# tristanGIANDO/python_ray_tracer

Measured on AMD Instinct MI355X. Metric: Mpixels/sec @1920x1080, 3 reflection bounces, higher is better.
Workload: dtype f64; 1 GPU; C2: README scene (BASELINE configs[1]) 1920x1080, 3 bounces; width=1920, height=1080, max_bounces=3, spheres=3, output=f32, mode=frames, parallelism=framesx1

## Files before the change

python_ray_tracer_amd/csrc/rtx_device.h:

```cpp
#pragma once

#include <hip/hip_ext.h>
#include <hip/hip_runtime.h>

#include <cstdint>
#include <cstdio>
#include <cstdlib>
#include <cstring>

#include "../../include/rtx_hip.h"
#include "rtx_internal.h"

#define FARAWAY 1.0e39
#define RTX_PI 3.141592653589793

namespace {

constexpr int kBlock = 256;
constexpr int kWaveW = 8;
constexpr int kWaveWSmall = 16;
constexpr int kFastWaves = 4;
constexpr int kFastWavesSmall = 1;
constexpr int kPersistMinSpheres = 32;
constexpr int kMaxFetch = 32;
constexpr int kDeferredWorkers = 4096;
constexpr int kDeepWorkers = 16384;
constexpr int kDeepWaves = 4;
constexpr int kDeepWavesTile = 5;
constexpr int kFwdWavesPersist = 4;
constexpr int kFwdWaves = 5;
constexpr int kFwdWavesLarge = 6;
constexpr int64_t kWavesLargeMinPixels = int64_t(4) << 20;
constexpr int kFwdWavesSmall = 5;
constexpr int kDeepLevels = 5;
constexpr int kCappedMax = RTX_FAST_MAX_BOUNCES;
constexpr int kShadeMath = 3;
constexpr int kWaveH = 64 / kWaveW;
static_assert(kFastWaves == 1 || kFastWaves == 2 || kFastWaves == 4, "kFastWaves");
static_assert(kFastWavesSmall == 1 || kFastWavesSmall == 2 || kFastWavesSmall == 4, "kFastWavesSmall");
static_assert((kMaxFetch & (kMaxFetch - 1)) == 0, "kMaxFetch must be a power of two");
constexpr int kFastBlock = 64 * kFastWaves;
constexpr int kWavesX = kFastWavesSmall == 1 ? 1 : 2;
constexpr int kWavesXTree = kFastWaves;
static_assert(kWaveWSmall > 0 && kWaveWSmall <= 64 && 64 % kWaveWSmall == 0, "kWaveWSmall");
template <bool TREE>
__host__ __device__ constexpr int wave_w() { return TREE ? kWaveW : kWaveWSmall; }
template <bool TREE>
__host__ __device__ constexpr int waves_x() { return TREE ? kWavesXTree : kWavesX; }
template <bool TREE>
__host__ __device__ constexpr int fast_waves() { return TREE ? kFastWaves : kFastWavesSmall; }
template <bool TREE>
// ... 40 lines not shown
  int64_t n_workers;
  int stack_levels;
  unsigned long long* stats;
  int n_tiles_x, n_tiles_y;
  uint32_t* fetch;
  int n_fetch;
  int64_t scene_stride;
  int n_frames;
  int frame;
  uint32_t* deferred_out;
  int no_general;
  int images;
  const uint32_t* tile_order;
  uint32_t* tile_cost;
  int reserve;
};

constexpr int kFrameShift = 34;
constexpr int kRaysShift = 50;
constexpr int kHitsShift = 57;
constexpr int kLevelMask = 0x7F;
constexpr int kRecWords = 10;
constexpr int kFirstPassLevels = 30;
constexpr int kDeepLevel3 = 60;
static_assert(kFirstPassLevels >= kDeepLevels && kFirstPassLevels < kDeepLevel3, "first-pass record level");
static_assert(kDeepLevel3 + 2 < kLevelMask, "deferred-entry level fields hold 7 bits");
constexpr int64_t records_cap(int64_t n, bool cont) {
  const int64_t lo = int64_t(1) << (cont ? 14 : 18);
  const int64_t by_n = n / (cont ? 2048 : 32);
  const int64_t want = by_n > lo ? by_n : lo;
// ... 19 lines not shown
}

__device__ __forceinline__ Params frame_view(const Params& p, int f) {
  Params q = p;
  q.scene = p.scene + (int64_t)f * p.scene_stride;
  q.out = (uint8_t*)p.out + (int64_t)f * p.n * out_bytes_per_pixel(p.out_kind);
  q.frame = f;
  return q;
}


__device__ __forceinline__ double dot3(double ax, double ay, double az, double bx, double by, double bz) {
  return ((ax * bx) + (ay * by)) + (az * bz);
}

__device__ __forceinline__ double sqrt_core(double x) {
  const double y = __builtin_amdgcn_rsq(x);
  double g = x * y;
  double h = y * 0.5;
  const double r = __builtin_fma(-h, g, 0.5);
  g = __builtin_fma(g, r, g);
  h = __builtin_fma(h, r, h);
  double d = __builtin_fma(-g, g, x);
  g = __builtin_fma(d, h, g);
  d = __builtin_fma(-g, g, x);
  return __builtin_fma(d, h, g);
}
__device__ __forceinline__ double sqrt_cr(double x) {
  if (__ballot(!(x >= 0x1.0p-767 && x <= 0x1.fffffffffffffp+1023)) == 0) return sqrt_core(x);
  return __builtin_sqrt(x);
// ... 6 lines not shown
  r = __builtin_fma(r, e, r);
  const double q = a * r;
  const double rem = __builtin_fma(-b, q, a);
  return __builtin_fma(rem, r, q);
}
__device__ __forceinline__ bool div_range(double x) {
  const double ax = fabs(x);
  return ax >= 0x1.0p-300 && ax <= 0x1.0p+300;
}
__device__ __forceinline__ double div_cr(double a, double b) {
  if (__ballot(!(div_range(b) && (a == 0.0 || div_range(a)))) == 0)
    return a == 0.0 ? a * __builtin_copysign(1.0, b) : div_core(a, b);
  return a / b;
}

__device__ __forceinline__ double inv_mag(double d) {
  if (__ballot(!(d >= 0x1.0p-600 && d <= 0x1.0p+600)) == 0) return div_core(1.0, sqrt_core(d));
  const double mag = sqrt_cr(d);
  return div_cr(1.0, mag == 0.0 ? 1.0 : mag);
}

__device__ __forceinline__ void norm3(double& x, double& y, double& z) {
  const double r = inv_mag(dot3(x, y, z, x, y, z));
  x = x * r;
  y = y * r;
  z = z * r;
}

__device__ __forceinline__ double inv_mag_near1(double d) {
  return __builtin_fma(-__builtin_floor((d - 1.0) * 0x1.0p51), 0x1.0p-52, 1.0);
}
__device__ __forceinline__ double inv_mag_unit(double d) {
  if (__ballot(!(fabs(d - 1.0) <= 0x1.0p-30)) == 0) return inv_mag_near1(d);
  return inv_mag(d);
}
__device__ __forceinline__ void norm3_unit(double& x, double& y, double& z) {
  const double r = inv_mag_unit(dot3(x, y, z, x, y, z));
  x = x * r;
  y = y * r;
  z = z * r;
}

__device__ __forceinline__ double clip01(double x) { return __builtin_fmin(__builtin_fmax(x, 0.0), 1.0); }

__device__ __forceinline__ double max0(double x) { return __builtin_fmax(x, 0.0); }

__device__ __forceinline__ int trunc_parity(double x) {
  const double k = trunc(x);
  const double h = k * 0.5;
  return (x == x) && (h != trunc(h));
}

// ... 12 lines not shown
  if (disc > 0.0 && !behind(b, c)) {
    const double sq = sqrt_cr(disc);
    const double s0 = (-b - sq) * 0.5;
    const double s1 = (-b + sq) * 0.5;
    const double sol = s0 > 0.0 ? s0 : s1;
    if (sol > 0.0) t = sol;
  }
  return t;
}

struct SphTest {
  double h, d;
  bool skip;
  int half;
};
__device__ __forceinline__ SphTest sph_test(double h, double c, double tame) {
  SphTest t;
  t.half = __ballot(!(fabs(h) >= tame)) == 0 ? 1 : 0;
  t.h = h;
  if (t.half) {
    t.d = (h * h) - c;
    t.skip = !(t.d > 0.0) || (h > 0.0 && c >= 0.0);
  } else {
    const double b = 2.0 * h;
    t.d = (b * b) - (4.0 * c);
    t.skip = !(t.d > 0.0) || behind(b, c);
  }
  return t;
}
template <typename P>
__device__ __forceinline__ SphTest isect_disc(const P* g, double ox, double oy, double oz, double oo, double dx,
                                              double dy, double dz, double tame) {
  const double cx = g[RTX_G_CX], cy = g[RTX_G_CY], cz = g[RTX_G_CZ];
  const double h = dot3(dx, dy, dz, ox - cx, oy - cy, oz - cz);
  const double c = ((g[RTX_G_CC] + oo) - 2.0 * dot3(cx, cy, cz, ox, oy, oz)) - g[RTX_G_RR];
  return sph_test(h, c, tame);
}
template <typename P>
__device__ __forceinline__ SphTest isect_disc_cam(const P* g, double ox, double oy, double oz, double dx, double dy,
                                                  double dz, double tame) {
  const double h = dot3(dx, dy, dz, ox - g[RTX_G_CX], oy - g[RTX_G_CY], oz - g[RTX_G_CZ]);
  return sph_test(h, g[RTX_G_C0], tame);
}
__device__ __forceinline__ double isect_sol(const SphTest& t, bool& valid) {
  if (t.half) {
    const double sq = sqrt_core(fabs(t.d));
    valid = !t.skip && sq > t.h;
    const uint32_t hi = __double2hiint(sq), lo = __double2loint(sq);
    const uint32_t shi = (-t.h > sq) ? (hi ^ 0x80000000u) : hi;
    return -t.h + __hiloint2double(shi, lo);
  }
  const double b = 2.0 * t.h;
  const double sq = sqrt_cr(fabs(t.d));
  const double s0 = (-b - sq) * 0.5;
  const double s1 = (-b + sq) * 0.5;
// ... 5 lines not shown
  if (!a.skip) {
    bool v;
    const double t = isect_sol(a, v);
    f(t, v);
  }
}
template <typename F>
__device__ __forceinline__ void isect_pair(const SphTest& a, const SphTest& b, F&& f) {
  if (!a.skip || !b.skip) {
    bool v0, v1;
    const double t0 = isect_sol(a, v0);
    const double t1 = isect_sol(b, v1);
    f(t0, v0, t1, v1);
  }
}
template <typename P>
__device__ __forceinline__ double isect_t(const P* g, double ox, double oy, double oz, double oo, double dx, double dy,
                                          double dz, double tame) {
  double r = FARAWAY;
  isect_one(isect_disc(g, ox, oy, oz, oo, dx, dy, dz, tame), [&](double t, bool v) {
    if (v) r = t;
  });
  return r;
}

__device__ __forceinline__ void nearest_update(bool valid, double t, int s, double& tmin, int& hit, bool& tie) {
  if (valid && t < tmin) {
    tmin = t;
    hit = s;
    tie = false;
  } else if (valid && t == tmin) {
    tie = true;
  }
// ... 193 lines not shown
          const cdouble* g0 = cg + __builtin_amdgcn_readfirstlane(k) * RTX_GEOM_WORDS;
          isect_one(isect_disc(g0, qx, qy, qz, qq, lx, ly, lz, tame), [&](double t0, bool v0) {
            if (v0 && t0 < tself) lit = false;
          });
        }
      }
      if (__ballot(lit) == 0) break;
      ++i;
    } else {
      i = (int)nd[RTX_N_SKIP];
    }
  }
  return lit;
}

template <bool CAM, typename P, typename Wk>
__device__ __forceinline__ void nearest_hit(const P* geo, int nsph, double ox, double oy, double oz, double dx,
                                            double dy, double dz, double& tmin, int& hit, bool& tie, double tame,
                                            Wk& wk) {
  wk.test(nsph);
  tmin = FARAWAY;
  hit = -1;
  tie = false;
  const double oo = CAM ? 0.0 : dot3(ox, oy, oz, ox, oy, oz);
  scan_range(
      geo, 0, nsph,
      [&](const P* g) {
        return CAM ? isect_disc_cam(g, ox, oy, oz, dx, dy, dz, tame) : isect_disc(g, ox, oy, oz, oo, dx, dy, dz, tame);
      },
      [](const P*, int s) { return s; }, [&](int s, double t, bool v) { nearest_update(v, t, s, tmin, hit, tie); });
}

__device__ __forceinline__ double sin_reduced(double x) {
// ... 3 lines not shown
  r = __builtin_fma(-n, -0x1.f1976b7ed8fbcp-109, r);
  const double z = r * r;
  double q = 0x1.71b8ef6dcf572p-66;
  q = __builtin_fma(z, q, -0x1.2f49b46814157p-57);
  q = __builtin_fma(z, q, 0x1.952c77030ad4ap-49);
  q = __builtin_fma(z, q, -0x1.ae7f3e733b81fp-41);
  q = __builtin_fma(z, q, 0x1.6124613a86d09p-33);
  q = __builtin_fma(z, q, -0x1.ae64567f544e4p-26);
  q = __builtin_fma(z, q, 0x1.71de3a556c734p-19);
  q = __builtin_fma(z, q, -0x1.a01a01a01a01ap-13);
  q = __builtin_fma(z, q, 0x1.1111111111111p-7);
  q = __builtin_fma(z, q, -0x1.5555555555555p-3);
  const double s = __builtin_fma(r * z, q, r);
  return ((int)n & 1) ? -s : s;
}
__device__ __forceinline__ double sin_ref(const cdouble* sc, double x) {
  if (sc[RTX_H_SINRED] != 0.0 || __ballot(!(fabs(x) <= 0x1.0p20)) == 0) return sin_reduced(x);
  return sin(x);
}

__device__ __forceinline__ double div_shade(double a, double b) {
  if constexpr (kShadeMath == 0) return div_cr(a, b);
  if constexpr (kShadeMath == 1) return div_core(a, b);
  double r = __builtin_amdgcn_rcp(b);
  r = __builtin_fma(r, __builtin_fma(-b, r, 1.0), r);
  r = __builtin_fma(r, __builtin_fma(-b, r, 1.0), r);
  return a * r;
}
__device__ __forceinline__ double sqrt_shade(double x) {
  if constexpr (kShadeMath == 0) return sqrt_cr(x);
  if constexpr (kShadeMath == 1) return x == 0.0 ? 0.0 : sqrt_core(x);
// ... 48 lines not shown
}

struct Hit {
  double dli;
  double di;
  double spec;
  double va;
  double g;
  int h;
  int tk;
  bool lit;
  double qx, qy, qz;
  double nx, ny, nz;
};

template <typename M>
__device__ __forceinline__ double specular(const M* mh, double g, double nx, double ny, double nz, double lx,
                                           double ly, double lz, double vx, double vy, double vz) {
  double Lx = lx, Ly = ly, Lz = lz;
  norm3_unit(Lx, Ly, Lz);
  double Vx = vx, Vy = vy, Vz = vz;
  norm3_unit(Vx, Vy, Vz);
  double Hx = Lx + Vx, Hy = Ly + Vy, Hz = Lz + Vz;
  {
    const double dh = dot3(Hx, Hy, Hz, Hx, Hy, Hz);
    const double rh = kShadeMath == 4 ? inv_mag_shade(dh) : inv_mag_shade_v(dh);
    Hx = Hx * rh;
    Hy = Hy * rh;
    Hz = Hz * rh;
  }
  const double NdotV = clip01(dot3(nx, ny, nz, Vx, Vy, Vz));
  if (!(NdotV > 0.0)) return 0.0;
  const double NdotH = clip01(dot3(nx, ny, nz, Hx, Hy, Hz));
  const double VdotH = clip01(dot3(Vx, Vy, Vz, Hx, Hy, Hz));
  const double NdotL = clip01(dot3(nx, ny, nz, Lx, Ly, Lz));
  const double F = __builtin_fma(mh[RTX_M_1MF0], pow5(1.0 - VdotH), mh[RTX_M_F0]);
  const double a2 = mh[RTX_M_A2];
  const double denom = (NdotH * NdotH) * mh[RTX_M_A2M1] + 1.0;
  const double Dd = RTX_PI * __builtin_fma(denom, denom, 1e-8);
  const double oma2 = mh[RTX_M_1MA2];
  const double dL = (NdotL + sqrt_shade(__builtin_fma(oma2, NdotL * NdotL, a2))) + 1e-8;
  const double dV = (NdotV + sqrt_shade(__builtin_fma(oma2, NdotV * NdotV, a2))) + 1e-8;
  const double spec_base = ((F * a2) * ((2.0 * NdotL) * (2.0 * NdotV))) *
                           div_shade(1.0, (dL * dV) * (Dd * __builtin_fma(4.0, NdotV, 1e-8)));
  const double glint = pow25(1.0 - NdotV) * NdotL;
  const double sf = __builtin_fma(g, glint, spec_base);
  return (NdotV <= 0.0) ? 0.0 : sf;
}

template <bool IMG = false, typename M>
__device__ __forceinline__ void hit_color(const M* mh, const cdouble* sc, double dli, double di, int tk, bool lit,
                                          bool weighted, double spec, double va, double Rr, double Rg, double Rb,
                                          double& cr, double& cg, double& cb) {
  const double litf = lit ? 1.0 : 0.0;
  double tr, tg, tb;
  const double tex = mh[RTX_M_TEX];
  if (tex == RTX_TEX_CHECKER) {
    tr = tg = tb = tk ? 1.0 : 0.0;
  } else if (IMG && tex == RTX_TEX_IMAGE) {
    const cdouble* t = sc + ((int64_t)mh[RTX_M_TR] + 3 * (int64_t)tk);
    tr = t[0];
    tg = t[1];
    tb = t[2];
  } else {
    tr = mh[RTX_M_TR];
    tg = mh[RTX_M_TG];
    tb = mh[RTX_M_TB];
  }
  const double dg = mh[RTX_M_DG];
  const double ar = __builtin_fma(sc[RTX_H_DOMEC + 0], di, __builtin_fma((tr * dli) * litf, dg, 0.004));
  const double ag = __builtin_fma(sc[RTX_H_DOMEC + 1], di, __builtin_fma((tg * dli) * litf, dg, 0.004));
  const double ab = __builtin_fma(sc[RTX_H_DOMEC + 2], di, __builtin_fma((tb * dli) * litf, dg, 0.004));
  const double g = mh[RTX_M_G];
  const double xr = weighted ? (spec + Rr * 0.5) * g : 0.0;
  const double xg = weighted ? (spec + Rg * 0.5) * g : 0.0;
  const double xb = weighted ? (spec + Rb * 0.5) * g : 0.0;
  double ir = 0.0, ig = 0.0, ib = 0.0;
  const double igain = mh[RTX_M_IG];
  if (igain != 0.0) {
    const double af = fabs(va - 0.5) * 2.0;
    const double phase = ((af * RTX_PI) * mh[RTX_M_TFT]) * 10.0;
    const double ip = sin_ref(sc, phase);
    const double hs = mh[RTX_M_HS], omhs = mh[RTX_M_1MHS];
    const double r = __builtin_fma(ip, hs, omhs * (1.0 - ip));
    const double gg = __builtin_fma(ip, omhs, hs * (1.0 - ip));
    const double b = __builtin_fma(0.5, ip, 0.5);
    const double w = mh[RTX_M_TFW];
    ir = (r * w) * igain;
    ig = (gg * w) * igain;
    ib = (b * w) * igain;
  }
  cr = (ar + xr) + ir;
  cg = (ag + xg) + ig;
  cb = (ab + xb) + ib;
}

constexpr int kGridWaterfall = 16;
// ... 53 lines not shown
                   [&](double t0, bool v0, double t1, bool v1) {
                     if (v0) tsh = __builtin_fmin(tsh, t0);
                     if (v1) tsh = __builtin_fmin(tsh, t1);
                     anyv = anyv || v0 || v1;
                   });
      } else {
        isect_one(a0, [&](double t0, bool v0) {
          if (v0) tsh = __builtin_fmin(tsh, t0);
          anyv = anyv || v0;
        });
      }
    }
  }
}

template <bool IMG = false, bool TREE = true, typename T, typename G, typename Wk>
__device__ __forceinline__ void shade(const cdouble* sc, const G* geo, const T* tab, int nsph, int h, double ox,
                                      double oy, double oz, double dx, double dy, double dz, double t, Hit& s,
                                      double tame, Wk& wk, const T* mat = nullptr) {
  const T* gh = tab + h * RTX_GEOM_WORDS;
  const T* mh = mat ? mat : tab + nsph * RTX_GEOM_WORDS + h * RTX_MAT_WORDS;
  const double px = ox + dx * t, py = oy + dy * t, pz = oz + dz * t;
  const double inv_r = gh[RTX_G_INVR];
  const double nx = (px - gh[RTX_G_CX]) * inv_r;
  const double ny = (py - gh[RTX_G_CY]) * inv_r;
  const double nz = (pz - gh[RTX_G_CZ]) * inv_r;
  double lx = sc[RTX_H_LIGHT + 0] - px, ly = sc[RTX_H_LIGHT + 1] - py, lz = sc[RTX_H_LIGHT + 2] - pz;
  norm3(lx, ly, lz);
  const double qx = px + nx * 0.0001, qy = py + ny * 0.0001, qz = pz + nz * 0.0001;

  const double qq = dot3(qx, qy, qz, qx, qy, qz);
  const int h0 = __builtin_amdgcn_readfirstlane(h);
  const int hs = __ballot(h != h0) == 0 ? h0 : nsph;
  bool lit = true;
  uint64_t m0, m1;
  if (TREE && sc[RTX_H_SHGRID] != 0.0 && sc[RTX_H_TAME] != 0.0 &&
      grid_mask(sc, qx, qy, qz, qq, lx, ly, lz, dot3(nx, ny, nz, nx, ny, nz), hs, m0, m1)) {
    wk.node();
    if ((m0 | m1) != 0) {
      double tsh;
      bool anyv;
      min_masked(geo, m0, m1, qx, qy, qz, qq, lx, ly, lz, tame, tsh, anyv, wk);
      if (__ballot(anyv) != 0) {
        const double tself = isect_t(gh, qx, qy, qz, qq, lx, ly, lz, tame);
        wk.test(1);
        lit = !(anyv && tsh < tself);
      }
    }
  } else if (!TREE && sc[RTX_H_TAME] != 0.0) {
    const int nshadow = nsph - (hs < nsph);
    double tsh = FARAWAY;
    bool anyv = false;
    int j = 0;
    for (; j + 1 < nshadow; j += 2) {
      const G* g0 = geo + __builtin_amdgcn_readfirstlane(j + (j >= hs)) * RTX_GEOM_WORDS;
      const G* g1 = geo + __builtin_amdgcn_readfirstlane(j + 1 + (j + 1 >= hs)) * RTX_GEOM_WORDS;
      wk.test(2);
      isect_pair(isect_disc(g0, qx, qy, qz, qq, lx, ly, lz, tame), isect_disc(g1, qx, qy, qz, qq, lx, ly, lz, tame),
                 [&](double t0, bool v0, double t1, bool v1) {
                   if (v0) tsh = __builtin_fmin(tsh, t0);
                   if (v1) tsh = __builtin_fmin(tsh, t1);
                   anyv = anyv || v0 || v1;
                 });
    }
// ... 50 lines not shown
  double di = 0.0;
  for (int j = 0; j < ndome; ++j) di = di + sc[RTX_H_DOMEI + j] * max0(up);

  const double g = mh[RTX_M_G];
  const bool weighted = lit && g != 0.0;
  const bool need_irid = mh[RTX_M_IG] != 0.0;
  double spec = 0.0, va = 0.0;
  if (weighted || need_irid) {
    double vx = sc[RTX_H_CAM + 0] - px, vy = sc[RTX_H_CAM + 1] - py, vz = sc[RTX_H_CAM + 2] - pz;
    {
      const double rv = inv_mag_shade_v(dot3(vx, vy, vz, vx, vy, vz));
      vx = vx * rv;
      vy = vy * rv;
      vz = vz * rv;
    }
    if (weighted) spec = specular(mh, g, nx, ny, nz, lx, ly, lz, vx, vy, vz);
    if (need_irid) va = clip01(dot3(nx, ny, nz, vx, vy, vz));
  }
  s.dli = dli;
  s.di = di;
  s.spec = spec;
  s.va = va;
  s.g = g;
  s.h = h;
  const double tex = mh[RTX_M_TEX];
  s.tk = tex == RTX_TEX_CHECKER ? (trunc_parity(px * 2.0) == trunc_parity(pz * 2.0))
         : tex != RTX_TEX_IMAGE ? 0
         : IMG ? image_texel(mh, gh, px, py, pz) : -1;
  s.lit = lit;
  s.qx = qx; s.qy = qy; s.qz = qz;
  s.nx = nx; s.ny = ny; s.nz = nz;
}

__device__ __forceinline__ void reflect_dir(double& dx, double& dy, double& dz, double nx, double ny, double nz) {
  const double dn = dot3(dx, dy, dz, nx, ny, nz);
  double rx = dx - (nx * 2.0) * dn, ry = dy - (ny * 2.0) * dn, rz = dz - (nz * 2.0) * dn;
  norm3_unit(rx, ry, rz);
  dx = rx;
  dy = ry;
  dz = rz;
}


__device__ __forceinline__ int global_row(const Params& p, int lr) {
  if (p.n_parts == 1) return lr;
  const int own = p.row_block * p.part_run;
  return (lr / own) * (p.n_parts * p.row_block) + p.part * p.row_block + (lr % own);
}

__device__ __forceinline__ void camera_dir(const cdouble* sc, int col, int r, int W, int H, double& dx, double& dy,
                                           double& dz) {
  const double x = (sc[RTX_H_XFIX] != 0.0 && col == W - 1) ? sc[RTX_H_XSTOP]
                                                            : (double)col * sc[RTX_H_XSTEP] + sc[RTX_H_XSTART];
  const double y = (sc[RTX_H_YFIX] != 0.0 && r == H - 1) ? sc[RTX_H_YSTOP]
                                                          : (double)r * sc[RTX_H_YSTEP] + sc[RTX_H_YSTART];
  const double vx = x - sc[RTX_H_CAM + 0];
  const double vy = y - sc[RTX_H_CAM + 1];
  const double vz = sc[RTX_H_VZ];
  const double rr = inv_mag(((vx * vx) + (vy * vy)) + sc[RTX_H_VZ2]);
  dx = vx * rr;
  dy = vy * rr;
  dz = vz * rr;
}

__device__ __forceinline__ void camera_ray(const Params& p, int col, int lr, double& ox, double& oy, double& oz,
                                           double& dx, double& dy, double& dz) {
  const cdouble* sc = (const cdouble*)p.scene;
  camera_dir(sc, col, global_row(p, lr), p.width, p.height, dx, dy, dz);
  ox = sc[RTX_H_CAM + 0];
  oy = sc[RTX_H_CAM + 1];
  oz = sc[RTX_H_CAM + 2];
}

__device__ __forceinline__ int huge_tail(const cdouble* sc, int nsph) {
  const int nb = (int)sc[RTX_H_NBEAM];
  return nb > 0 && nb < nsph ? nb : nsph;
}

__device__ __forceinline__ bool wave_frustum(const Params& p, int c0, int lr0, uint64_t& m0, uint64_t& m1) {
  const cdouble* sc = (const cdouble*)p.scene;
  const int W = p.width;
  if (c0 >= W || lr0 >= p.n_rows) return false;
  const int c1 = c0 + kWaveW - 1 < W - 1 ? c0 + kWaveW - 1 : W - 1;
// ... 244 lines not shown
    o[1] = quant_u8(g);
    o[2] = quant_u8(b);
  }
}

__device__ __forceinline__ void stat_add(unsigned long long* st, int word, unsigned long long v) {
  atomicAdd(st + word, v);
}

__device__ __forceinline__ void stat_wave(unsigned long long* st, int word) {
  const unsigned long long m = __ballot(1);
  if ((int)__lane_id() == __ffsll((long long)m) - 1) atomicAdd(st + word, 1ull);
}


template <int B, bool LDS, int DEEP, bool STATS, bool TREE, bool BEAM, bool IMG = false, int NSPH = 0>
__device__ __forceinline__ void fast_tile(const Params& p, int bx, int by, bool first, const double* lds_tab,
                                          bool wave_tile = false) {
  constexpr int FB = fast_block<TREE>();
  const cdouble* sc = (const cdouble*)p.scene;
  const cdouble* geo = sc + RTX_HDR_WORDS;
  const int nsph = NSPH > 0 ? NSPH : p.nsph;
  const int nb = TREE ? huge_tail(sc, nsph) : nsph;
  const double tame = p.mode != 1 && p.mode != 3 && sc[RTX_H_TAME] != 0.0 ? 0x1.0p-350 : __builtin_nan("");

  int64_t i = 0;
  bool active;
  int kb = 0;
  const double* rin = nullptr;
  int col = 0, lr = 0;
  constexpr int WW = wave_w<TREE>(), WH = 64 / WW, WX = waves_x<TREE>(), WY = fast_waves<TREE>() / WX;
  const int wv = __builtin_amdgcn_readfirstlane((int)(threadIdx.x >> 6));
  auto pixel_index = [&](int lane) -> int64_t {
    if (p.mode == 0) {
      const int c = wave_tile ? bx * WW + (lane % WW) : bx * (WX * WW) + (wv % WX) * WW + (lane % WW);
      const int r = wave_tile ? by * WH + (lane / WW) : by * (WY * WH) + (wv / WX) * WH + (lane / WW);
      return (int64_t)r * p.width + c;
    }
    return (int64_t)bx * FB + wv * 64 + lane;
// ... 33 lines not shown
  uint64_t fm0 = 0, fm1 = 0;
  bool fr = false;
  if constexpr (TREE) {
    if (cam0 && nsph <= 128 && sc[RTX_H_NNODES] != 0.0 && sc[RTX_H_SBOX] != 0.0 && sc[RTX_H_TAME] != 0.0 &&
        sc[RTX_H_VZ] != 0.0) {
      const int lane = threadIdx.x & 63;
      fr = wave_frustum(p, __builtin_amdgcn_readfirstlane(col - lane % kWaveW),
                        __builtin_amdgcn_readfirstlane(lr - lane / kWaveW), fm0, fm1);
    }
  }
  if (active) {
    if (rin) {
      ox = rin[0]; oy = rin[1]; oz = rin[2];
      dx = rin[3]; dy = rin[4]; dz = rin[5];
    } else if (cam0) {
      camera_ray(p, col, lr, ox, oy, oz, dx, dy, dz);
    } else {
      load_ray(p, i, ox, oy, oz, dx, dy, dz);
    }
    if (st) {
      if (!rin) stat_add(st, RTX_S_PIXELS, 1);
      if (kb < RTX_S_LEVELS) {
        stat_add(st, RTX_S_RAYS + kb, 1);
        stat_wave(st, RTX_S_WTRACE + kb);
      }
    }
    if (p.mode == 3) {
      tmin = p.hit_t[i];
      hit = p.hit_shape;
      tie = sc[RTX_H_MAT0] != 0.0;
    } else if (TREE && sc[RTX_H_NNODES] != 0.0) {
      if (fr) {
        nearest_masked<true>(geo, fm0, fm1, ox, oy, oz, dx, dy, dz, tmin, hit, tie, tame, wk);
      } else if (cam0) {
        nearest_bvh<true>(sc, ox, oy, oz, dx, dy, dz, tmin, hit, tie, tame, wk);
      } else {
        nearest_bvh<false>(sc, ox, oy, oz, dx, dy, dz, tmin, hit, tie, tame, wk);
      }
    } else if (cam0) {
      nearest_hit<true>(geo, nsph, ox, oy, oz, dx, dy, dz, tmin, hit, tie, tame, wk);
    } else {
      nearest_hit<false>(geo, nsph, ox, oy, oz, dx, dy, dz, tmin, hit, tie, tame, wk);
    }
  }
  if constexpr (LDS) {
    if (first) __syncthreads();
  }
  if (!active) return;
  constexpr bool CL = !DEEP && LDS && TREE && !BEAM;
  static_assert(!CL || 3 * sizeof(double) * FB == kColourLdsBytes, "colour LDS");
  double* const cl = CL ? const_cast<double*>(lds_tab) + nsph * kSphWords + threadIdx.x : nullptr;
  if constexpr (CL) {
    cl[0] = 0.0;
    cl[FB] = 0.0;
    cl[2 * FB] = 0.0;
  }

  double cr = 0.0, cg = 0.0, cb = 0.0;
  double thr = 1.0;
  if constexpr (DEEP == 2) {
    if (rin) {
      cr = rin[6];
      cg = rin[7];
// ... 23 lines not shown
      deferred = true;
      rays_through = kb + k;
      hits_through = kb + k - 1;
      break;
    }
    if (st && kb + k < RTX_S_LEVELS) {
      stat_add(st, RTX_S_HITS + kb + k, 1);
      stat_wave(st, RTX_S_WSHADE + kb + k);
    }
    const bool weighted = s.lit && s.g != 0.0;
    const bool at_cap = DEEP && p.max_bounces >= 0 && kb + k >= p.max_bounces;
    {
      const double* tab = LDS ? (const double*)lds_tab : p.scene + RTX_HDR_WORDS;
      double lr_, lg_, lb_;
      hit_color<IMG>(tab + nsph * RTX_GEOM_WORDS + hit * RTX_MAT_WORDS, sc, s.dli, s.di, s.tk, s.lit, weighted, s.spec,
                     s.va, 0.0, 0.0, 0.0, lr_, lg_, lb_);
      if constexpr (CL) {
        cl[0] = __builtin_fma(thr, lr_, cl[0]);
        cl[FB] = __builtin_fma(thr, lg_, cl[FB]);
        cl[2 * FB] = __builtin_fma(thr, lb_, cl[2 * FB]);
      } else {
        cr = __builtin_fma(thr, lr_, cr);
        cg = __builtin_fma(thr, lg_, cg);
        cb = __builtin_fma(thr, lb_, cb);
      }
      const int kmax = DEEP ? p.drec_level - kb : B;
      if (DEEP && weighted && k >= kmax && !at_cap) {
        deferred = true;
        appended = true;
        rays_through = hits_through = kb + kmax;
        const int64_t slot = append_deferred(p, deferred_entry(DEEP == 2 || !TREE ? i : pixel_index(lane_id_fresh()),
                                                               p.frame, kb + kmax, kb + kmax));
        if (p.drec && slot >= 0 && slot < p.rec_cap) {
          double* rec = p.drec + slot * kRecWords;
          double rx = dx, ry = dy, rz = dz;
          reflect_dir(rx, ry, rz, s.nx, s.ny, s.nz);
          rec[0] = s.qx; rec[1] = s.qy; rec[2] = s.qz;
          rec[3] = rx; rec[4] = ry; rec[5] = rz;
          rec[6] = cr; rec[7] = cg; rec[8] = cb;
          rec[9] = (thr * 0.5) * s.g;
        }
        break;
      }
      if (!weighted || k >= kmax || at_cap) break;
      thr = (thr * 0.5) * s.g;
    }
    reflect_dir(dx, dy, dz, s.nx, s.ny, s.nz);
    ox = s.qx;
    oy = s.qy;
    oz = s.qz;
    if (st && kb + k + 1 < RTX_S_LEVELS) {
      stat_add(st, RTX_S_RAYS + kb + k + 1, 1);
      stat_wave(st, RTX_S_WTRACE + kb + k + 1);
    }
    [[maybe_unused]] uint32_t tests0 = 0, nodes0 = 0;
    if constexpr (STATS) {
      tests0 = wk.tests;
      nodes0 = wk.nodes;
    }
    if (TREE && sc[RTX_H_NNODES] != 0.0) {
      Beam bm;
      const double* btab = LDS ? (const double*)lds_tab : p.scene + RTX_HDR_WORDS;
// ... 11 lines not shown
      wk.tests1 += wk.tests - tests0;
      wk.nodes1 += wk.nodes - nodes0;
    }
  }

  if constexpr (STATS) {
    if (st) {
      stat_add(st, RTX_S_TESTS, wk.tests);
      stat_add(st, RTX_S_NODES, wk.nodes);
      stat_add(st, RTX_S_TESTS1, wk.tests1);
      stat_add(st, RTX_S_NODES1, wk.nodes1);
      stat_add(st, RTX_S_BOXES, wk.boxes);
      stat_add(st, RTX_S_BEAMT, wk.beamt);
    }
  }
  const int64_t io = DEEP == 2 || !TREE ? i : pixel_index(lane_id_fresh());
  if constexpr (CL) {
    cr = cl[0];
    cg = cl[FB];
    cb = cl[2 * FB];
  }
  if (deferred) {
    if (!appended) append_deferred(p, deferred_entry(io, p.frame, rays_through, hits_through));
    if (st && !rin) stat_add(st, RTX_S_DEFERRED, 1);
    return;
  }
  write_out(p, io, cr, cg, cb);
}

template <int B, bool LDS, int DEEP, bool STATS, int TP, bool IMG, int NSPH>
__device__ __forceinline__ void k_render_fast_tiles(const Params& p, const double* lds_tab);

template <int B, bool LDS, int DEEP, bool STATS = false, int TP = 2, bool IMG = false, int NSPH = 0, int WAVES = 0>
__global__ __launch_bounds__(fast_block<(TP >= 1)>(),
                             WAVES > 0 ? WAVES
                             : DEEP    ? (TP >= 2 || DEEP == 2 ? kDeepWaves : kDeepWavesTile)
                                       : (TP >= 2 ? kFwdWavesPersist : TP ? kFwdWaves : kFwdWavesSmall)) void
k_render_fast(Params p0) {
  constexpr bool TREE = TP >= 1;
  constexpr bool BEAM = TP >= 2;
  extern __shared__ double lds_tab[];
  const Params p = frame_view(p0, blockIdx.z);
  {
    const cdouble* sc = (const cdouble*)p.scene;
    if (sc[RTX_H_MAGIC] != RTX_MAGIC || sc[RTX_H_NSPH] != (double)p.nsph || (NSPH > 0 && p.nsph != NSPH)) {
      if (threadIdx.x == 0) atomicOr((uint32_t*)p.ws + RTX_WS_STATUS, (uint32_t)RTX_ST_BAD_SCENE);
      return;
    }
  }
  if constexpr (LDS) {
    const double* src = p.scene + RTX_HDR_WORDS;
    for (int k = threadIdx.x; k < p.nsph * kSphWords; k += fast_block<TREE>()) {
      const bool bw = BEAM && kBeamStaged && k < p.nsph * RTX_GEOM_WORDS && (k & (RTX_GEOM_WORDS - 1)) == RTX_G_IDX;
      lds_tab[k] = bw ? beam_word(src[k - RTX_G_IDX + RTX_G_CC], src[k - RTX_G_IDX + RTX_G_RR]) : src[k];
    }
  }
  if constexpr (DEEP == 2) {
// ... 47 lines not shown
    return;
  }
  const uint64_t t_entry = STATS && p.tile_cost ? __builtin_amdgcn_s_memrealtime() : 0;
  int bx = blockIdx.x, by = gridDim.y - 1 - blockIdx.y, tb = blockIdx.y * gridDim.x + blockIdx.x;
  if (p.tile_order) {
    tb = (int)((const uint32_t __attribute__((address_space(4)))*)p.tile_order)[tb];
    if ((unsigned)tb >= gridDim.x * gridDim.y) return;
    bx = tb % gridDim.x;
    by = gridDim.y - 1 - tb / gridDim.x;
  }
  fast_tile<B, LDS, DEEP, STATS, TREE, BEAM, IMG, NSPH>(p, bx, by, true, lds_tab);
  if (STATS && p.tile_cost && (threadIdx.x & 63) == 0)
    atomicMax(p.tile_cost + tb, (uint32_t)(__builtin_amdgcn_s_memrealtime() - t_entry));
}

}
```

python_ray_tracer_amd/csrc/rtx_small.hip:

```cpp
#include "rtx_device.h"
#include "rtx_internal.h"

namespace {

template <int B, int DEEP, bool STATS, bool IMG = false, int NSPH = 0>
hipError_t go(const void* params, dim3 grid, uint32_t lds, hipStream_t s, hipEvent_t e0, hipEvent_t e1) {
  const Params& p = *static_cast<const Params*>(params);
  rtx_note_launch(B, true, DEEP, STATS, 0, IMG, NSPH, 0, grid, p.n_fetch, p.tile_order != nullptr, lds);
  hipExtLaunchKernelGGL((k_render_fast<B, true, DEEP, STATS, 0, IMG, NSPH>), grid, dim3(fast_block<false>()), lds, s,
                        e0, e1, 0u, p);
  return hipSuccess;
}

template <int B, int DEEP>
hipError_t go_ns(const void* params, dim3 grid, uint32_t lds, hipStream_t s, hipEvent_t e0, hipEvent_t e1) {
  static_assert(kTreeMinSpheres == 8, "one instantiation per sphere count 1..7");
  switch (static_cast<const Params*>(params)->nsph) {
    case 1: return go<B, DEEP, false, false, 1>(params, grid, lds, s, e0, e1);
    case 2: return go<B, DEEP, false, false, 2>(params, grid, lds, s, e0, e1);
    case 3: return go<B, DEEP, false, false, 3>(params, grid, lds, s, e0, e1);
    case 4: return go<B, DEEP, false, false, 4>(params, grid, lds, s, e0, e1);
    case 5: return go<B, DEEP, false, false, 5>(params, grid, lds, s, e0, e1);
    case 6: return go<B, DEEP, false, false, 6>(params, grid, lds, s, e0, e1);
    case 7: return go<B, DEEP, false, false, 7>(params, grid, lds, s, e0, e1);
// ... 35 lines not shown
```

Before: 42320 Mpixels/s.

## Add optimistic small-scene wave path with sticky range guards and deferred LDS staging

Adds a dedicated small_wave path for single-wave small-scene kernels. It runs an optimistic tile body in which the per-call wave ballots for range checks (sqrt/div/normalise, sphere test, sine reduction) become a sticky per-lane flag; if any lane trips it, the whole tile is recomputed with the exact path. Scene table words are preloaded into registers and written to LDS only when some lane actually hits a sphere, and tile_order decoding uses a precomputed reciprocal instead of division. This trades fewer ballots and branches for higher register pressure, more code, and a possible full redo on rare inputs.

```diff
diff --git a/python_ray_tracer_amd/csrc/rtx_device.h b/python_ray_tracer_amd/csrc/rtx_device.h
--- a/python_ray_tracer_amd/csrc/rtx_device.h
+++ b/python_ray_tracer_amd/csrc/rtx_device.h
@@ -7,6 +7,7 @@
 #include <cstdio>
 #include <cstdlib>
 #include <cstring>
+#include <type_traits>
 
 #include "../../include/rtx_hip.h"
 #include "rtx_internal.h"
@@ -35,6 +36,8 @@
 constexpr int kDeepLevels = 5;
 constexpr int kCappedMax = RTX_FAST_MAX_BOUNCES;
 constexpr int kShadeMath = 3;
+constexpr bool kSmallOptimistic = true;
+constexpr bool kSmallLateStage = true;
 constexpr int kWaveH = 64 / kWaveW;
 static_assert(kFastWaves == 1 || kFastWaves == 2 || kFastWaves == 4, "kFastWaves");
 static_assert(kFastWavesSmall == 1 || kFastWavesSmall == 2 || kFastWavesSmall == 4, "kFastWavesSmall");
@@ -105,6 +108,7 @@
   const uint32_t* tile_order;
   uint32_t* tile_cost;
   int reserve;
+  uint32_t tile_div;
 };
 
 constexpr int kFrameShift = 34;
@@ -154,6 +158,14 @@
   return ((ax * bx) + (ay * by)) + (az * bz);
 }
 
+struct Sticky {
+  bool& bad;
+  __device__ __forceinline__ operator double() const { return 0x1.0p-350; }
+  __device__ __forceinline__ void trip(bool failed) const { bad = bad || failed; }
+};
+template <typename Tm>
+constexpr bool kSticky = std::is_same<Tm, Sticky>::value;
+
 __device__ __forceinline__ double sqrt_core(double x) {
   const double y = __builtin_amdgcn_rsq(x);
   double g = x * y;
@@ -190,14 +202,20 @@
   return a / b;
 }
 
-__device__ __forceinline__ double inv_mag(double d) {
+template <typename Tm = double>
+__device__ __forceinline__ double inv_mag(double d, Tm tame = Tm()) {
+  if constexpr (kSticky<Tm>) {
+    tame.trip(!(d >= 0x1.0p-600 && d <= 0x1.0p+600));
+    return div_core(1.0, sqrt_core(d));
+  }
   if (__ballot(!(d >= 0x1.0p-600 && d <= 0x1.0p+600)) == 0) return div_core(1.0, sqrt_core(d));
   const double mag = sqrt_cr(d);
   return div_cr(1.0, mag == 0.0 ? 1.0 : mag);
 }
 
-__device__ __forceinline__ void norm3(double& x, double& y, double& z) {
-  const double r = inv_mag(dot3(x, y, z, x, y, z));
+template <typename Tm = double>
+__device__ __forceinline__ void norm3(double& x, double& y, double& z, Tm tame = Tm()) {
+  const double r = inv_mag(dot3(x, y, z, x, y, z), tame);
   x = x * r;
   y = y * r;
   z = z * r;
@@ -206,12 +224,18 @@
 __device__ __forceinline__ double inv_mag_near1(double d) {
   return __builtin_fma(-__builtin_floor((d - 1.0) * 0x1.0p51), 0x1.0p-52, 1.0);
 }
-__device__ __forceinline__ double inv_mag_unit(double d) {
+template <typename Tm = double>
+__device__ __forceinline__ double inv_mag_unit(double d, Tm tame = Tm()) {
+  if constexpr (kSticky<Tm>) {
+    tame.trip(!(fabs(d - 1.0) <= 0x1.0p-30));
+    return inv_mag_near1(d);
+  }
   if (__ballot(!(fabs(d - 1.0) <= 0x1.0p-30)) == 0) return inv_mag_near1(d);
   return inv_mag(d);
 }
-__device__ __forceinline__ void norm3_unit(double& x, double& y, double& z) {
-  const double r = inv_mag_unit(dot3(x, y, z, x, y, z));
+template <typename Tm = double>
+__device__ __forceinline__ void norm3_unit(double& x, double& y, double& z, Tm tame = Tm()) {
+  const double r = inv_mag_unit(dot3(x, y, z, x, y, z), tame);
   x = x * r;
   y = y * r;
   z = z * r;
@@ -254,9 +278,15 @@
   bool skip;
   int half;
 };
-__device__ __forceinline__ SphTest sph_test(double h, double c, double tame) {
+template <typename Tm>
+__device__ __forceinline__ SphTest sph_test(double h, double c, Tm tame) {
   SphTest t;
-  t.half = __ballot(!(fabs(h) >= tame)) == 0 ? 1 : 0;
+  if constexpr (kSticky<Tm>) {
+    tame.trip(!(fabs(h) >= 0x1.0p-350));
+    t.half = 1;
+  } else {
+    t.half = __ballot(!(fabs(h) >= tame)) == 0 ? 1 : 0;
+  }
   t.h = h;
   if (t.half) {
     t.d = (h * h) - c;
@@ -268,17 +298,17 @@
   }
   return t;
 }
-template <typename P>
+template <typename P, typename Tm>
 __device__ __forceinline__ SphTest isect_disc(const P* g, double ox, double oy, double oz, double oo, double dx,
-                                              double dy, double dz, double tame) {
+                                              double dy, double dz, Tm tame) {
   const double cx = g[RTX_G_CX], cy = g[RTX_G_CY], cz = g[RTX_G_CZ];
   const double h = dot3(dx, dy, dz, ox - cx, oy - cy, oz - cz);
   const double c = ((g[RTX_G_CC] + oo) - 2.0 * dot3(cx, cy, cz, ox, oy, oz)) - g[RTX_G_RR];
   return sph_test(h, c, tame);
 }
-template <typename P>
+template <typename P, typename Tm>
 __device__ __forceinline__ SphTest isect_disc_cam(const P* g, double ox, double oy, double oz, double dx, double dy,
-                                                  double dz, double tame) {
+                                                  double dz, Tm tame) {
   const double h = dot3(dx, dy, dz, ox - g[RTX_G_CX], oy - g[RTX_G_CY], oz - g[RTX_G_CZ]);
   return sph_test(h, g[RTX_G_C0], tame);
 }
@@ -314,9 +344,9 @@
     f(t0, v0, t1, v1);
   }
 }
-template <typename P>
+template <typename P, typename Tm>
 __device__ __forceinline__ double isect_t(const P* g, double ox, double oy, double oz, double oo, double dx, double dy,
-                                          double dz, double tame) {
+                                          double dz, Tm tame) {
   double r = FARAWAY;
   isect_one(isect_disc(g, ox, oy, oz, oo, dx, dy, dz, tame), [&](double t, bool v) {
     if (v) r = t;
@@ -540,9 +570,9 @@
   return lit;
 }
 
-template <bool CAM, typename P, typename Wk>
+template <bool CAM, typename P, typename Wk, typename Tm>
 __device__ __forceinline__ void nearest_hit(const P* geo, int nsph, double ox, double oy, double oz, double dx,
-                                            double dy, double dz, double& tmin, int& hit, bool& tie, double tame,
+                                            double dy, double dz, double& tmin, int& hit, bool& tie, Tm tame,
                                             Wk& wk) {
   wk.test(nsph);
   tmin = FARAWAY;
@@ -576,7 +606,12 @@
   const double s = __builtin_fma(r * z, q, r);
   return ((int)n & 1) ? -s : s;
 }
-__device__ __forceinline__ double sin_ref(const cdouble* sc, double x) {
+template <typename Tm = double>
+__device__ __forceinline__ double sin_ref(const cdouble* sc, double x, Tm tame = Tm()) {
+  if constexpr (kSticky<Tm>) {
+    tame.trip(!(sc[RTX_H_SINRED] != 0.0 || fabs(x) <= 0x1.0p20));
+    return sin_reduced(x);
+  }
   if (sc[RTX_H_SINRED] != 0.0 || __ballot(!(fabs(x) <= 0x1.0p20)) == 0) return sin_reduced(x);
   return sin(x);
 }
@@ -655,13 +690,13 @@
   double nx, ny, nz;
 };
 
-template <typename M>
+template <typename M, typename Tm = double>
 __device__ __forceinline__ double specular(const M* mh, double g, double nx, double ny, double nz, double lx,
-                                           double ly, double lz, double vx, double vy, double vz) {
+                                           double ly, double lz, double vx, double vy, double vz, Tm tame = Tm()) {
   double Lx = lx, Ly = ly, Lz = lz;
-  norm3_unit(Lx, Ly, Lz);
+  norm3_unit(Lx, Ly, Lz, tame);
   double Vx = vx, Vy = vy, Vz = vz;
-  norm3_unit(Vx, Vy, Vz);
+  norm3_unit(Vx, Vy, Vz, tame);
   double Hx = Lx + Vx, Hy = Ly + Vy, Hz = Lz + Vz;
   {
     const double dh = dot3(Hx, Hy, Hz, Hx, Hy, Hz);
@@ -689,10 +724,10 @@
   return (NdotV <= 0.0) ? 0.0 : sf;
 }
 
-template <bool IMG = false, typename M>
+template <bool IMG = false, typename M, typename Tm = double>
 __device__ __forceinline__ void hit_color(const M* mh, const cdouble* sc, double dli, double di, int tk, bool lit,
                                           bool weighted, double spec, double va, double Rr, double Rg, double Rb,
-                                          double& cr, double& cg, double& cb) {
+                                          double& cr, double& cg, double& cb, Tm tame = Tm()) {
   const double litf = lit ? 1.0 : 0.0;
   double tr, tg, tb;
   const double tex = mh[RTX_M_TEX];
@@ -721,7 +756,7 @@
   if (igain != 0.0) {
     const double af = fabs(va - 0.5) * 2.0;
     const double phase = ((af * RTX_PI) * mh[RTX_M_TFT]) * 10.0;
-    const double ip = sin_ref(sc, phase);
+    const double ip = sin_ref(sc, phase, tame);
     const double hs = mh[RTX_M_HS], omhs = mh[RTX_M_1MHS];
     const double r = __builtin_fma(ip, hs, omhs * (1.0 - ip));
     const double gg = __builtin_fma(ip, omhs, hs * (1.0 - ip));
@@ -805,10 +840,10 @@
   }
 }
 
-template <bool IMG = false, bool TREE = true, typename T, typename G, typename Wk>
+template <bool IMG = false, bool TREE = true, typename T, typename G, typename Wk, typename Tm>
 __device__ __forceinline__ void shade(const cdouble* sc, const G* geo, const T* tab, int nsph, int h, double ox,
                                       double oy, double oz, double dx, double dy, double dz, double t, Hit& s,
-                                      double tame, Wk& wk, const T* mat = nullptr) {
+                                      Tm tame, Wk& wk, const T* mat = nullptr) {
   const T* gh = tab + h * RTX_GEOM_WORDS;
   const T* mh = mat ? mat : tab + nsph * RTX_GEOM_WORDS + h * RTX_MAT_WORDS;
   const double px = ox + dx * t, py = oy + dy * t, pz = oz + dz * t;
@@ -817,7 +852,7 @@
   const double ny = (py - gh[RTX_G_CY]) * inv_r;
   const double nz = (pz - gh[RTX_G_CZ]) * inv_r;
   double lx = sc[RTX_H_LIGHT + 0] - px, ly = sc[RTX_H_LIGHT + 1] - py, lz = sc[RTX_H_LIGHT + 2] - pz;
-  norm3(lx, ly, lz);
+  norm3(lx, ly, lz, tame);
   const double qx = px + nx * 0.0001, qy = py + ny * 0.0001, qz = pz + nz * 0.0001;
 
   const double qq = dot3(qx, qy, qz, qx, qy, qz);
@@ -838,7 +873,7 @@
         lit = !(anyv && tsh < tself);
       }
     }
-  } else if (!TREE && sc[RTX_H_TAME] != 0.0) {
+  } else if (!TREE && (kSticky<Tm> || sc[RTX_H_TAME] != 0.0)) {
     const int nshadow = nsph - (hs < nsph);
     double tsh = FARAWAY;
     bool anyv = false;
@@ -919,7 +954,7 @@
       vy = vy * rv;
       vz = vz * rv;
     }
-    if (weighted) spec = specular(mh, g, nx, ny, nz, lx, ly, lz, vx, vy, vz);
+    if (weighted) spec = specular(mh, g, nx, ny, nz, lx, ly, lz, vx, vy, vz, tame);
     if (need_irid) va = clip01(dot3(nx, ny, nz, vx, vy, vz));
   }
   s.dli = dli;
@@ -937,10 +972,12 @@
   s.nx = nx; s.ny = ny; s.nz = nz;
 }
 
-__device__ __forceinline__ void reflect_dir(double& dx, double& dy, double& dz, double nx, double ny, double nz) {
+template <typename Tm = double>
+__device__ __forceinline__ void reflect_dir(double& dx, double& dy, double& dz, double nx, double ny, double nz,
+                                            Tm tame = Tm()) {
   const double dn = dot3(dx, dy, dz, nx, ny, nz);
   double rx = dx - (nx * 2.0) * dn, ry = dy - (ny * 2.0) * dn, rz = dz - (nz * 2.0) * dn;
-  norm3_unit(rx, ry, rz);
+  norm3_unit(rx, ry, rz, tame);
   dx = rx;
   dy = ry;
   dz = rz;
@@ -953,8 +990,9 @@
   return (lr / own) * (p.n_parts * p.row_block) + p.part * p.row_block + (lr % own);
 }
 
+template <typename Tm = double>
 __device__ __forceinline__ void camera_dir(const cdouble* sc, int col, int r, int W, int H, double& dx, double& dy,
-                                           double& dz) {
+                                           double& dz, Tm tame = Tm()) {
   const double x = (sc[RTX_H_XFIX] != 0.0 && col == W - 1) ? sc[RTX_H_XSTOP]
                                                             : (double)col * sc[RTX_H_XSTEP] + sc[RTX_H_XSTART];
   const double y = (sc[RTX_H_YFIX] != 0.0 && r == H - 1) ? sc[RTX_H_YSTOP]
@@ -962,16 +1000,17 @@
   const double vx = x - sc[RTX_H_CAM + 0];
   const double vy = y - sc[RTX_H_CAM + 1];
   const double vz = sc[RTX_H_VZ];
-  const double rr = inv_mag(((vx * vx) + (vy * vy)) + sc[RTX_H_VZ2]);
+  const double rr = inv_mag(((vx * vx) + (vy * vy)) + sc[RTX_H_VZ2], tame);
   dx = vx * rr;
   dy = vy * rr;
   dz = vz * rr;
 }
 
+template <typename Tm = double>
 __device__ __forceinline__ void camera_ray(const Params& p, int col, int lr, double& ox, double& oy, double& oz,
-                                           double& dx, double& dy, double& dz) {
+                                           double& dx, double& dy, double& dz, Tm tame = Tm()) {
   const cdouble* sc = (const cdouble*)p.scene;
-  camera_dir(sc, col, global_row(p, lr), p.width, p.height, dx, dy, dz);
+  camera_dir(sc, col, global_row(p, lr), p.width, p.height, dx, dy, dz, tame);
   ox = sc[RTX_H_CAM + 0];
   oy = sc[RTX_H_CAM + 1];
   oz = sc[RTX_H_CAM + 2];
@@ -1246,15 +1285,20 @@
 }
 
 
-template <int B, bool LDS, int DEEP, bool STATS, bool TREE, bool BEAM, bool IMG = false, int NSPH = 0>
-__device__ __forceinline__ void fast_tile(const Params& p, int bx, int by, bool first, const double* lds_tab,
-                                          bool wave_tile = false) {
+template <int B, bool LDS, int DEEP, bool STATS, bool TREE, bool BEAM, bool IMG = false, int NSPH = 0,
+          typename Tm, typename Stage>
+__device__ __forceinline__ bool fast_tile_body(const Params& p, int bx, int by, const double* lds_tab,
+                                               bool wave_tile, Tm guard, Stage&& stage) {
+  static_assert(!kSticky<Tm> || (DEEP == 0 && !TREE && !STATS), "the optimistic body: capped, counter-free, TP 0");
   constexpr int FB = fast_block<TREE>();
   const cdouble* sc = (const cdouble*)p.scene;
   const cdouble* geo = sc + RTX_HDR_WORDS;
   const int nsph = NSPH > 0 ? NSPH : p.nsph;
   const int nb = TREE ? huge_tail(sc, nsph) : nsph;
-  const double tame = p.mode != 1 && p.mode != 3 && sc[RTX_H_TAME] != 0.0 ? 0x1.0p-350 : __builtin_nan("");
+  const auto tame = [&] {
+    if constexpr (kSticky<Tm>) return guard;
+    else return p.mode != 1 && p.mode != 3 && sc[RTX_H_TAME] != 0.0 ? 0x1.0p-350 : __builtin_nan("");
+  }();
 
   int64_t i = 0;
   bool active;
@@ -1318,7 +1362,7 @@
       ox = rin[0]; oy = rin[1]; oz = rin[2];
       dx = rin[3]; dy = rin[4]; dz = rin[5];
     } else if (cam0) {
-      camera_ray(p, col, lr, ox, oy, oz, dx, dy, dz);
+      camera_ray(p, col, lr, ox, oy, oz, dx, dy, dz, tame);
     } else {
       load_ray(p, i, ox, oy, oz, dx, dy, dz);
     }
@@ -1347,10 +1391,10 @@
       nearest_hit<false>(geo, nsph, ox, oy, oz, dx, dy, dz, tmin, hit, tie, tame, wk);
     }
   }
-  if constexpr (LDS) {
-    if (first) __syncthreads();
-  }
-  if (!active) return;
+  stage(hit);
+  if constexpr (!kSticky<Tm>) {
+    if (!active) return false;
+  }
   constexpr bool CL = !DEEP && LDS && TREE && !BEAM;
   static_assert(!CL || 3 * sizeof(double) * FB == kColourLdsBytes, "colour LDS");
   double* const cl = CL ? const_cast<double*>(lds_tab) + nsph * kSphWords + threadIdx.x : nullptr;
@@ -1404,7 +1448,7 @@
       const double* tab = LDS ? (const double*)lds_tab : p.scene + RTX_HDR_WORDS;
       double lr_, lg_, lb_;
       hit_color<IMG>(tab + nsph * RTX_GEOM_WORDS + hit * RTX_MAT_WORDS, sc, s.dli, s.di, s.tk, s.lit, weighted, s.spec,
-                     s.va, 0.0, 0.0, 0.0, lr_, lg_, lb_);
+                     s.va, 0.0, 0.0, 0.0, lr_, lg_, lb_, tame);
       if constexpr (CL) {
         cl[0] = __builtin_fma(thr, lr_, cl[0]);
         cl[FB] = __builtin_fma(thr, lg_, cl[FB]);
@@ -1435,7 +1479,7 @@
       if (!weighted || k >= kmax || at_cap) break;
       thr = (thr * 0.5) * s.g;
     }
-    reflect_dir(dx, dy, dz, s.nx, s.ny, s.nz);
+    reflect_dir(dx, dy, dz, s.nx, s.ny, s.nz, tame);
     ox = s.qx;
     oy = s.qy;
     oz = s.qz;
@@ -1477,6 +1521,10 @@
       stat_add(st, RTX_S_BEAMT, wk.beamt);
     }
   }
+  if constexpr (kSticky<Tm>) {
+    if (__ballot(guard.bad) != 0) return true;
+    if (!active) return false;
+  }
   const int64_t io = DEEP == 2 || !TREE ? i : pixel_index(lane_id_fresh());
   if constexpr (CL) {
     cr = cl[0];
@@ -1486,13 +1534,26 @@
   if (deferred) {
     if (!appended) append_deferred(p, deferred_entry(io, p.frame, rays_through, hits_through));
     if (st && !rin) stat_add(st, RTX_S_DEFERRED, 1);
-    return;
+    return false;
   }
   write_out(p, io, cr, cg, cb);
+  return false;
+}
+
+template <int B, bool LDS, int DEEP, bool STATS, bool TREE, bool BEAM, bool IMG = false, int NSPH = 0>
+__device__ __forceinline__ void fast_tile(const Params& p, int bx, int by, bool first, const double* lds_tab,
+                                          bool wave_tile = false) {
+  fast_tile_body<B, LDS, DEEP, STATS, TREE, BEAM, IMG, NSPH>(p, bx, by, lds_tab, wave_tile, 0.0, [&](int) {
+    if constexpr (LDS) {
+      if (first) __syncthreads();
+    }
+  });
 }
 
 template <int B, bool LDS, int DEEP, bool STATS, int TP, bool IMG, int NSPH>
 __device__ __forceinline__ void k_render_fast_tiles(const Params& p, const double* lds_tab);
+template <int B, int DEEP, bool STATS, bool IMG, int NSPH>
+__device__ __forceinline__ void small_wave(const Params& p, double* lds_tab);
 
 template <int B, bool LDS, int DEEP, bool STATS = false, int TP = 2, bool IMG = false, int NSPH = 0, int WAVES = 0>
 __global__ __launch_bounds__(fast_block<(TP >= 1)>(),
@@ -1504,6 +1565,11 @@
   constexpr bool BEAM = TP >= 2;
   extern __shared__ double lds_tab[];
   const Params p = frame_view(p0, blockIdx.z);
+  if constexpr (TP == 0 && DEEP != 2) {
+    static_assert(LDS, "the small-scene kernels stage the table in LDS");
+    small_wave<B, DEEP, STATS, IMG, NSPH>(p, lds_tab);
+    return;
+  }
   {
     const cdouble* sc = (const cdouble*)p.scene;
     if (sc[RTX_H_MAGIC] != RTX_MAGIC || sc[RTX_H_NSPH] != (double)p.nsph || (NSPH > 0 && p.nsph != NSPH)) {
@@ -1581,4 +1647,102 @@
     atomicMax(p.tile_cost + tb, (uint32_t)(__builtin_amdgcn_s_memrealtime() - t_entry));
 }
 
-}
+constexpr int kSmallStage = ((kTreeMinSpheres - 1) * kSphWords + 63) / 64;
+template <int B, int DEEP, bool STATS, bool IMG, int NSPH>
+__device__ __forceinline__ void small_wave(const Params& p, double* lds_tab) {
+  static_assert(kFastWavesSmall == 1 && fast_block<false>() == 64, "small_wave: one wave per block");
+  static_assert(DEEP != 2, "the continuation pass is k_render_fast's");
+  const uint64_t t_entry = STATS && p.tile_cost ? __builtin_amdgcn_s_memrealtime() : 0;
+  const cdouble* sc = (const cdouble*)p.scene;
+  const double magic = sc[RTX_H_MAGIC], hn = sc[RTX_H_NSPH];
+  constexpr int NL = NSPH > 0 ? (NSPH * kSphWords + 63) / 64 : kSmallStage;
+  const double* src = p.scene + RTX_HDR_WORDS;
+  const int nw0 = p.nsph * kSphWords;
+  const int lane = threadIdx.x;
+  double tv[NL];
+  if constexpr (kSmallLateStage) {
+#pragma unroll
+    for (int j = 0; j < NL; ++j) tv[j] = lane + 64 * j < nw0 ? src[lane + 64 * j] : 0.0;
+  }
+  uint32_t tb = blockIdx.y * gridDim.x + blockIdx.x;
+  if constexpr (kSmallLateStage) {
+    const uint32_t gy = gridDim.y;
+    asm volatile("" ::"s"(p.tile_div), "s"(gy), "s"(p.n), "s"(p.part_run), "s"(p.out), "s"(p.no_general));
+  }
+  if (p.tile_order) tb = ((const uint32_t __attribute__((address_space(4)))*)p.tile_order)[tb];
+  if constexpr (kSmallLateStage) {
+    const double htame = sc[RTX_H_TAME], c0 = sc[RTX_H_CAM + 0], c1 = sc[RTX_H_CAM + 1], c2 = sc[RTX_H_CAM + 2];
+    const double x0 = sc[RTX_H_XSTART], x1 = sc[RTX_H_XSTEP], y0 = sc[RTX_H_YSTART], y1 = sc[RTX_H_YSTEP];
+    const double xf = sc[RTX_H_XFIX], yf = sc[RTX_H_YFIX];
+    const double vz = sc[RTX_H_VZ], vz2 = sc[RTX_H_VZ2];
+    if constexpr (NSPH >= 1 && NSPH <= 3) {
+      asm volatile("" ::"s"(magic), "s"(hn), "s"(htame), "s"(tb), "s"(c0), "s"(c1), "s"(c2), "s"(x0), "s"(x1), "s"(y0),
+                   "s"(y1), "s"(xf), "s"(yf), "s"(vz), "s"(vz2));
+    } else {
+      asm volatile("" ::"s"(magic), "s"(hn), "s"(htame), "s"(tb));
+    }
+  }
+  if (magic != RTX_MAGIC || hn != (double)p.nsph || (NSPH > 0 && p.nsph != NSPH)) {
+    if (threadIdx.x == 0) atomicOr((uint32_t*)p.ws + RTX_WS_STATUS, (uint32_t)RTX_ST_BAD_SCENE);
+    return;
+  }
+  const int nw = NSPH > 0 ? NSPH * kSphWords : nw0;
+  int bx = blockIdx.x, by = gridDim.y - 1 - blockIdx.y;
+  if (p.tile_order) {
+    if (tb >= gridDim.x * gridDim.y) return;
+    uint32_t q = __umulhi(tb, p.tile_div), r = tb - q * gridDim.x;
+    if (r >= gridDim.x) {
+      r -= gridDim.x;
+      ++q;
+    }
+    bx = (int)r;
+    by = (int)(gridDim.y - 1 - q);
+  }
+  bool staged = false;
+  if constexpr (!kSmallLateStage) {
+    for (int k = lane; k < nw; k += 64) lds_tab[k] = src[k];
+    __syncthreads();
+    staged = true;
+  }
+  auto stage_regs = [&](int hit) {
+    if constexpr (!kSmallLateStage) return;
+    if (nw > 64 * NL) {
+      for (int k = lane; k < nw; k += 64) lds_tab[k] = src[k];
+      __syncthreads();
+      staged = true;
+    } else if (__ballot(hit >= 0) != 0) {
+#pragma unroll
+      for (int j = 0; j < NL; ++j)
+        if (lane + 64 * j < nw) lds_tab[lane + 64 * j] = tv[j];
+      __syncthreads();
+      staged = true;
+    }
+  };
+  constexpr bool OPT = kSmallOptimistic && DEEP == 0 && !STATS && !IMG && NSPH > 0;
+  bool redo = true;
+  if constexpr (OPT) {
+    if (p.mode == 0 && sc[RTX_H_TAME] != 0.0) {
+      bool bad = false;
+      redo = fast_tile_body<B, true, DEEP, STATS, false, false, IMG, NSPH>(p, bx, by, lds_tab, false, Sticky{bad},
+                                                                          stage_regs);
+    }
+  }
+  if (redo) {
+    if constexpr (OPT) {
+      Params q = p;
+      asm volatile("" : "+s"(q.scene));
+      fast_tile_body<B, true, DEEP, STATS, false, false, IMG, NSPH>(q, bx, by, lds_tab, false, 0.0, [&](int hit) {
+        if (!staged && __ballot(hit >= 0) != 0) {
+          for (int k = lane; k < nw; k += 64) lds_tab[k] = src[k];
+          __syncthreads();
+        }
+      });
+    } else {
+      fast_tile_body<B, true, DEEP, STATS, false, false, IMG, NSPH>(p, bx, by, lds_tab, false, 0.0, stage_regs);
+    }
+  }
+  if (STATS && p.tile_cost && (threadIdx.x & 63) == 0)
+    atomicMax(p.tile_cost + tb, (uint32_t)(__builtin_amdgcn_s_memrealtime() - t_entry));
+}
+
+}
diff --git a/python_ray_tracer_amd/csrc/rtx_small.hip b/python_ray_tracer_amd/csrc/rtx_small.hip
--- a/python_ray_tracer_amd/csrc/rtx_small.hip
+++ b/python_ray_tracer_amd/csrc/rtx_small.hip
@@ -5,7 +5,8 @@
 
 template <int B, int DEEP, bool STATS, bool IMG = false, int NSPH = 0>
 hipError_t go(const void* params, dim3 grid, uint32_t lds, hipStream_t s, hipEvent_t e0, hipEvent_t e1) {
-  const Params& p = *static_cast<const Params*>(params);
+  Params p = *static_cast<const Params*>(params);
+  p.tile_div = grid.x > 1 ? (uint32_t)((uint64_t(1) << 32) / grid.x) : 0xFFFFFFFFu;
   rtx_note_launch(B, true, DEEP, STATS, 0, IMG, NSPH, 0, grid, p.n_fetch, p.tile_order != nullptr, lds);
   hipExtLaunchKernelGGL((k_render_fast<B, true, DEEP, STATS, 0, IMG, NSPH>), grid, dim3(fast_block<false>()), lds, s,
                         e0, e1, 0u, p);
```

New measurement: 45630 Mpixels/s, median of 6. 1.08x the previous value.
